# IuvenisSapiens/Qwen3-TTS-Rust

Hardware: AMD Instinct MI355X
Metric: audio-seconds generated per second (aggregate over GPUs) = concurrent real-time streams; RTF and first-chunk latency from the single-utterance leg (higher is better)
Workload: dtype i8

## Files before the change

### qwen3-tts-rust_amd/csrc/kernels.hip

```cpp
#include "kernels.h"
#include <cstdlib>
#include "q3_common.h"
#include "../../include/q3tts_spec.h"
#include "kdev.h"
#include "wslice.h"

namespace q3 {

Q3_STAMP_SETTER(set_stamp_buffer)

template <int LPR, int MT>
__global__ void __launch_bounds__(512) k_gemv_q8(Q8Mat w, int row0, int nrows, const int8_t* __restrict__ xq,
                                                 const uint16_t* __restrict__ xd, float* __restrict__ out,
                                                 int out_stride, int ntok) {
    constexpr int R = 64 / LPR, BPL = LPR / 2, NLD = 8 / BPL;
    __shared__ float red[8][R * MT];
    const int lane = threadIdx.x & 63, wave = threadIdx.x >> 6;
    const int r = lane % R, q = lane / R, half = q & 1, bil = q >> 1;
    const int nseg = w.K >> 8, nb = w.K >> 5;
    const int sseg = blockIdx.y, seg = sseg * 8 + wave;
    const int tok0 = blockIdx.z * MT;
    const bool active = seg < nseg;
    float acc[MT];
#pragma unroll
// ... 558 lines not shown
                asm volatile("" : "+v"(xl), "+v"(c) :: "memory");
                av[8 - NLATE + i] = *reinterpret_cast<const i32x4v*>(xl + (8 - NLATE + i) * 32);
            }
#pragma unroll
            for (int g4 = 0; g4 < 4; g4++) {
                const f32x2v sc_a = f32x2v{D[4 * g4], D[4 * g4 + 1]}, sc_b = f32x2v{D[4 * g4 + 2], D[4 * g4 + 3]};
                const f32x2v ca = f32x2v{(float)c[4 * g4], (float)c[4 * g4 + 1]}, cb = f32x2v{(float)c[4 * g4 + 2], (float)c[4 * g4 + 3]};
                acc2[2 * g4] = __builtin_elementwise_fma(ca, sc_a, acc2[2 * g4]);
                acc2[2 * g4 + 1] = __builtin_elementwise_fma(cb, sc_b, acc2[2 * g4 + 1]);
            }
        }
#pragma unroll
        for (int g = 0; g < 16; g++) red[wave][(g & 3) + 8 * (g >> 2) + 4 * half][r] = acc2[g >> 1][g & 1];
    };
    auto seg_sums = [&](int m, int c4) -> float4 {
        float4 v[4];
#pragma unroll
        for (int s2 = 0; s2 < 4; s2++) v[s2] = *reinterpret_cast<const float4*>(&red[s2][m][c4]);
        float4 S = v[0];
#pragma unroll
        for (int s2 = 1; s2 < 4; s2++)
            if (s2 < nsg) { S.x = S.x + v[s2].x; S.y = S.y + v[s2].y; S.z = S.z + v[s2].z; S.w = S.w + v[s2].w; }
        if (nsg > 4) {
            asm volatile("" ::: "memory");
#pragma unroll
            for (int s2 = 0; s2 < 4; s2++) v[s2] = *reinterpret_cast<const float4*>(&red[4 + s2][m][c4]);
#pragma unroll
            for (int s2 = 0; s2 < 4; s2++)
                if (4 + s2 < nsg) { S.x = S.x + v[s2].x; S.y = S.y + v[s2].y; S.z = S.z + v[s2].z; S.w = S.w + v[s2].w; }
        }
        return S;
    };
    const int nthr = 64 * (nseg < 8 ? nseg : 8);
    load_w(0, 0, 8);
    chain();
    Q3_STAMP(1);
    if (GU) { load_a(); load_w(1, 0, 8); }
    wg_barrier_lds();
    Q3_STAMP(2);
    if (!GU) {
        for (int t = threadIdx.x; t < 256; t += nthr) {
            const int m = t >> 3, c4 = (t & 7) * 4, tok = tok0 + m;
            const float4 S = seg_sums(m, c4);
            const int orow = blockIdx.x * 32 + c4;
            if (orow < nrows && tok < ntok) *reinterpret_cast<float4*>(out + ((size_t)sseg * ntok + tok) * out_stride + orow) = S;
        }
        Q3_STAMP(6);
        Q3_STAMP_FLUSH();
        return;
    }
    for (int t = threadIdx.x; t < 256; t += nthr) *reinterpret_cast<float4*>(&gate_s[4 * t]) = seg_sums(t >> 3, (t & 7) * 4);
    wg_barrier_lds();
    Q3_STAMP(3);
    chain();
    Q3_STAMP(4);
    wg_barrier_lds();
    Q3_STAMP(5);
    for (int t = threadIdx.x; t < 256; t += nthr) {
        const int m = t >> 3, c4 = (t & 7) * 4, tok = tok0 + m;
        const float4 U = seg_sums(m, c4), G = *reinterpret_cast<const float4*>(&gate_s[4 * t]);
        const float y0 = q3_swiglu(G.x, U.x), y1 = q3_swiglu(G.y, U.y), y2 = q3_swiglu(G.z, U.z), y3 = q3_swiglu(G.w, U.w);
        float amax = fmaxf(fmaxf(q3_fabsf(y0), q3_fabsf(y1)), fmaxf(q3_fabsf(y2), q3_fabsf(y3)));
        amax = fmaxf(amax, xor_lane<4>(amax)); amax = fmaxf(amax, xor_lane<2>(amax)); amax = fmaxf(amax, xor_lane<1>(amax));
        const float dd = amax / 127.0f;
        const float id = (dd != 0.0f) ? (1.0f / dd) : 0.0f;
        if (tok < ntok) {
            const uint32_t pk = ((uint32_t)(int)q3_rintf(y0 * id) & 0xFFu) | (((uint32_t)(int)q3_rintf(y1 * id) & 0xFFu) << 8) |
                                (((uint32_t)(int)q3_rintf(y2 * id) & 0xFFu) << 16) | (((uint32_t)(int)q3_rintf(y3 * id) & 0xFFu) << 24);
            *reinterpret_cast<uint32_t*>(aq + (size_t)tok * ff + blockIdx.x * 32 + c4) = pk;
            if (c4 == 0) ad[(size_t)tok * (ff >> 5) + blockIdx.x] = f2h(dd);
        }
    }
    Q3_STAMP(6);
    Q3_STAMP_FLUSH();
}

template <bool GU, int TS>
__global__ void __launch_bounds__(512) __attribute__((amdgpu_waves_per_eu(2, 2)))
k_gemm_kq_mfma(Q8Mat w, int row0, int nrows, const int8_t* __restrict__ xq, const uint16_t* __restrict__ xd, float* __restrict__ out, int out_stride,
               int ntok, int ff, int8_t* __restrict__ aq, uint16_t* __restrict__ ad) {
    __shared__ float red[8][32][33];
    __shared__ float gate_s[GU ? 4 : 1][GU ? 1024 : 1];
    const int lane = threadIdx.x & 63, wave = threadIdx.x >> 6;
    const int r = lane & 31, half = lane >> 5;
    const int nseg = w.K >> 8, nb = w.K >> 5;
    const int sseg = blockIdx.y, seg = sseg * 8 + wave;
    int nsg = nseg - sseg * 8;
    if (nsg > 8) nsg = 8;
    const bool active = seg < nseg;
    const int ntiles = (ntok + 31) >> 5;
    constexpr int NM = GU ? 2 : 1;
    const int row_first = row0 + blockIdx.x * 32;
    wslice_dispatch<TS>(w, (row_first > w.Npad - 1 ? w.Npad - 1 : row_first) >> 5, [&](auto tag) {
        constexpr int WT = decltype(tag)::value;
        constexpr bool Q5 = WT == Q3_T_Q5_K, Q6 = WT == Q3_T_Q6_K;
#pragma unroll 1
        for (int q = 0; q < NM; q++) {
            WSlice<2, WT> ws;
            ws.dwv = make_uint4(0, 0, 0, 0); ws.mv = make_uint4(0, 0, 0, 0);
            int row = row_first + r + q * ff;
            if (row > w.Npad - 1) row = w.Npad - 1;
            if (active) { ws.load(w, row >> 5, row & 31, seg, half, 0); ws.finish(half); }
            const float d0 = h2f(half_of(ws.dwv, 0)), d1 = h2f(half_of(ws.dwv, 1));
            int lt = 0;
#pragma unroll 1
            for (int tt = blockIdx.z; tt < ntiles; tt += gridDim.z, lt++) {
                const int tok0 = tt * 32;
                if (active) {
                    int atok = tok0 + r;
                    if (atok > ntok - 1) atok = ntok - 1;
                    const int8_t* xp = xq + (size_t)atok * w.K + seg * 256 + half * 16;
                    const uint4 dxa = *reinterpret_cast<const uint4*>(xd + (size_t)atok * nb + seg * 8);
                    float acc[16];
#pragma unroll
                    for (int g = 0; g < 16; g++) acc[g] = 0.0f;
                    const i32x4v ones = i32x4v{0x01010101, 0x01010101, 0x01010101, 0x01010101}, zero4 = i32x4v{0, 0, 0, 0};
#pragma unroll
                    for (int ip = 0; ip < 4; ip++) {
                        f32x32q D;
#pragma unroll
                        for (int g = 0; g < 32; g++) D[g] = 0.0f;
                        const uint32_t ex = half ? half_of(dxa, 2 * ip + 1) : half_of(dxa, 2 * ip);
                        D = __builtin_amdgcn_mfma_f32_32x32x1f32(h2f(ex), 1.0f, D, 0, 0, 0);
#pragma unroll
                        for (int i2 = 0; i2 < 2; i2++) {
                            const int i = 2 * ip + i2;
                            const i32x4v av = *reinterpret_cast<const i32x4v*>(xp + i * 32);
                            const i32x4v wv = i32x4v{(int)ws.wv[i].x, (int)ws.wv[i].y, (int)ws.wv[i].z, (int)ws.wv[i].w};
                            i32x16 z16;
#pragma unroll
                            for (int g = 0; g < 16; g++) z16[g] = 0;
                            if (Q5) {
                                const i32x16 c = __builtin_amdgcn_mfma_i32_32x32x32_i8(av, wv, z16, 0, 0, 0);
                                const i32x16 cx = __builtin_amdgcn_mfma_i32_32x32x32_i8(av, ones, z16, 0, 0, 0);
                                const int scb = ws.mbyte(i), mb = ws.mbyte(8 + i);
#pragma unroll
                                for (int g = 0; g < 16; g++) {
                                    const int i1 = __mul24(scb, c[g]), i2v = __mul24(mb, cx[g]);
                                    const float a = d0 * (float)i1;
                                    const float a2 = d1 * (float)i2v;
                                    const float diff = a - a2;
                                    acc[g] = q3_fmaf(diff, D[16 * i2 + g], acc[g]);
                                }
                            } else if (Q6) {
                                const i32x4v wlo = half ? zero4 : wv, whi = half ? wv : zero4, olo = half ? zero4 : ones, ohi = half ? ones : zero4;
                                const i32x16 clo = __builtin_amdgcn_mfma_i32_32x32x32_i8(av, wlo, z16, 0, 0, 0);
                                const i32x16 chi = __builtin_amdgcn_mfma_i32_32x32x32_i8(av, whi, z16, 0, 0, 0);
                                const i32x16 xlo = __builtin_amdgcn_mfma_i32_32x32x32_i8(av, olo, z16, 0, 0, 0);
                                const i32x16 xhi = __builtin_amdgcn_mfma_i32_32x32x32_i8(av, ohi, z16, 0, 0, 0);
                                const int s0 = (int)(int8_t)ws.mbyte(2 * i), s1 = (int)(int8_t)ws.mbyte(2 * i + 1);
#pragma unroll
                                for (int g = 0; g < 16; g++) {
                                    const int isum = __mul24(clo[g] - 32 * xlo[g], s0) + __mul24(chi[g] - 32 * xhi[g], s1);
                                    const float a = d0 * (float)isum;
                                    acc[g] = q3_fmaf(a, D[16 * i2 + g], acc[g]);
                                }
                            } else {
                                const i32x16 c = __builtin_amdgcn_mfma_i32_32x32x32_i8(av, wv, z16, 0, 0, 0);
                                const float dwf = h2f(half_of(ws.dwv, i));
#pragma unroll
                                for (int g = 0; g < 16; g++) acc[g] = q3_fmaf((float)c[g], dwf * D[16 * i2 + g], acc[g]);
                            }
                        }
                    }
#pragma unroll
                    for (int g = 0; g < 16; g++) red[wave][(g & 3) + 8 * (g >> 2) + 4 * half][r] = acc[g];
                }
                wg_barrier_lds();
                for (int t = threadIdx.x; t < 32 * 32; t += blockDim.x) {
                    const int m = t >> 5, rr = t & 31, tok = tok0 + m;
                    float v8[8];
#pragma unroll
                    for (int s2 = 0; s2 < 8; s2++) v8[s2] = red[s2][m][rr];
                    float S = v8[0];
#pragma unroll
                    for (int s2 = 1; s2 < 8; s2++) S = (s2 < nsg) ? S + v8[s2] : S;
                    if (!GU) {
                        const int orow = blockIdx.x * 32 + rr;
                        if (orow < nrows && tok < ntok) out[((size_t)sseg * ntok + tok) * out_stride + orow] = S;
                    } else if (q == 0) gate_s[lt][t] = S;
                    else {
                        const float y = q3_swiglu(gate_s[lt][t], S);
                        float amax = q3_fabsf(y);
                        amax = fmaxf(amax, xor_lane<16>(amax)); amax = fmaxf(amax, xor_lane<8>(amax)); amax = fmaxf(amax, xor_lane<4>(amax));
                        amax = fmaxf(amax, xor_lane<2>(amax)); amax = fmaxf(amax, xor_lane<1>(amax));
                        const float dd = amax / 127.0f;
                        const float id = (dd != 0.0f) ? (1.0f / dd) : 0.0f;
                        if (tok < ntok) {
                            aq[(size_t)tok * ff + blockIdx.x * 32 + rr] = (int8_t)(int)q3_rintf(y * id);
                            if (rr == 0) ad[(size_t)tok * (ff >> 5) + blockIdx.x] = f2h(dd);
                        }
                    }
                }
                wg_barrier_lds();
            }
        }
    });
}


__global__ void __launch_bounds__(64) k_rmsnorm_quant(NormArgs a) {
    const int tok = blockIdx.x, lane = threadIdx.x;
    const int nch = a.d >> 8;
    const float* hin = a.h_in;
    if (a.idx_keys) hin += (size_t)key_code(a.idx_keys[(size_t)tok * a.idx_stride]) * a.h_stride;
    else if (a.idx) hin += (size_t)a.idx[(size_t)tok * a.idx_stride] * a.h_stride;
    else hin += (size_t)tok * a.h_stride;
    float4 x[8];
    float p = 0.0f;
#pragma unroll
    for (int c = 0; c < 8; c++) {
        if (c < nch) {
            float4 v = *reinterpret_cast<const float4*>(hin + 256 * c + 4 * lane);
            if (a.nparts > 0) {
                const float* pp = a.parts + (size_t)tok * a.parts_stride + 256 * c + 4 * lane;
                float4 y = *reinterpret_cast<const float4*>(pp);
                for (int s = 1; s < a.nparts; s++) {
                    const float4 z = *reinterpret_cast<const float4*>(pp + (size_t)s * gridDim.x * a.parts_stride);
                    y.x = y.x + z.x; y.y = y.y + z.y; y.z = y.z + z.z; y.w = y.w + z.w;
                }
                v.x = v.x + y.x; v.y = v.y + y.y; v.z = v.z + y.z; v.w = v.w + y.w;
            }
            if (a.h_out) *reinterpret_cast<float4*>(a.h_out + (size_t)tok * a.d + 256 * c + 4 * lane) = v;
            x[c] = v;
            p = q3_fmaf(v.x, v.x, p); p = q3_fmaf(v.y, v.y, p); p = q3_fmaf(v.z, v.z, p); p = q3_fmaf(v.w, v.w, p);
        }
    }
    const float ss = wave_sum_bfly(p);
    const float mean = ss / (float)a.d;
    const float scale = 1.0f / q3_sqrtf(mean + a.eps);
#pragma unroll
    for (int c = 0; c < 8; c++) {
        if (c < nch) {
            const float4 g = *reinterpret_cast<const float4*>(a.g + 256 * c + 4 * lane);
            float4 y;
            y.x = (x[c].x * scale) * g.x; y.y = (x[c].y * scale) * g.y;
            y.z = (x[c].z * scale) * g.z; y.w = (x[c].w * scale) * g.w;
            if (a.xn_out) *reinterpret_cast<float4*>(a.xn_out + (size_t)tok * a.d + 256 * c + 4 * lane) = y;
            float amax = fmaxf(fmaxf(q3_fabsf(y.x), q3_fabsf(y.y)), fmaxf(q3_fabsf(y.z), q3_fabsf(y.w)));
            amax = fmaxf(amax, xor_lane<1>(amax)); amax = fmaxf(amax, xor_lane<2>(amax)); amax = fmaxf(amax, xor_lane<4>(amax));
            const float dd = amax / 127.0f;
            const float id = (dd != 0.0f) ? (1.0f / dd) : 0.0f;
            const int q0 = (int)q3_rintf(y.x * id), q1 = (int)q3_rintf(y.y * id), q2 = (int)q3_rintf(y.z * id), q3v = (int)q3_rintf(y.w * id);
            const uint32_t pk = (uint32_t)(q0 & 0xFF) | ((uint32_t)(q1 & 0xFF) << 8) | ((uint32_t)(q2 & 0xFF) << 16) | ((uint32_t)(q3v & 0xFF) << 24);
            *reinterpret_cast<uint32_t*>(a.xq + (size_t)tok * a.d + 256 * c + 4 * lane) = pk;
            if ((lane & 7) == 0) a.xd[(size_t)tok * (a.d >> 5) + 8 * c + (lane >> 3)] = f2h(dd);
        }
    }
}
void launch_rmsnorm_quant(hipStream_t st, const NormArgs& a, int ntok) {
    hipLaunchKernelGGL(k_rmsnorm_quant, dim3(ntok), dim3(64), 0, st, a);
}

__global__ void __launch_bounds__(64) k_qk_rope_append(QkvRows qkv, int n_head, int n_kv,
                                                       const float* __restrict__ q_norm_w, const float* __restrict__ k_norm_w,
                                                       float eps, const float* __restrict__ rope_cos,
                                                       const float* __restrict__ rope_sin, int n_ctx,
                                                       const int32_t* __restrict__ mrope_sec, TokMeta tm, KvCache kv,
                                                       int layer, float* __restrict__ qrot) {
    const int hv = blockIdx.x, tok = blockIdx.y, lane = threadIdx.x;
    const float* vec = qkv.row(tok) + (size_t)hv * 128;
    float x1 = vec[lane], x2 = vec[lane + 64];
    const int seq = tm.seq_of(tok), slot = tm.slot_of(tok);
    const int page = kv.page_of(seq, slot >> 6);
    const int ps = slot & 63;
    if (hv < n_head + n_kv) {
        const float* w = hv < n_head ? q_norm_w : k_norm_w;
        float p = x1 * x1;
        p = q3_fmaf(x2, x2, p);
        const float ss = wave_sum_bfly(p);
        const float mean = ss / 128.0f;
        const float scale = 1.0f / q3_sqrtf(mean + eps);
        const float y1 = (x1 * scale) * w[lane], y2 = (x2 * scale) * w[lane + 64];
        int32_t sec[4] = { mrope_sec[0], mrope_sec[1], mrope_sec[2], mrope_sec[3] };
        int pp = tm.pos_of(tok, q3_mrope_stream(lane, sec));
        if (pp < 0) pp = 0;
        if (pp > n_ctx - 1) pp = n_ctx - 1;
        float o1, o2;
        q3_rope_pair(y1, y2, rope_cos[(size_t)pp * 64 + lane], rope_sin[(size_t)pp * 64 + lane], &o1, &o2);
        if (hv < n_head) {
            float* dst = qrot + ((size_t)tok * n_head + hv) * 128;
            dst[lane] = o1; dst[lane + 64] = o2;
        } else {
            const int kh = hv - n_head;
            uint16_t* Kb = kv.k + (size_t)page * kv.page_stride() + (size_t)layer * kv.layer_stride() + (size_t)kh * 8192;
            Kb[((lane >> 3) * 64 + ps) * 8 + (lane & 7)] = f2h(o1);
            Kb[(((lane + 64) >> 3) * 64 + ps) * 8 + (lane & 7)] = f2h(o2);
        }
    } else {
        const int vh = hv - n_head - n_kv;
        uint16_t* Vb = kv.v + (size_t)page * kv.page_stride() + (size_t)layer * kv.layer_stride() + (size_t)vh * 8192;
        Vb[ps * 128 + lane] = f2h(x1);
        Vb[ps * 128 + lane + 64] = f2h(x2);
    }
}
void launch_qk_rope_append(hipStream_t st, const QkvRows& qkv, const float*, int n_head, int n_kv,
                           const float* q_norm_w, const float* k_norm_w, float eps, const float* rope_cos,
                           const float* rope_sin, int n_ctx, const int32_t* mrope_sec, const TokMeta& tm,
                           const KvCache& kv, int layer, float* qrot, int ntok) {
    hipLaunchKernelGGL(k_qk_rope_append, dim3(n_head + 2 * n_kv, ntok), dim3(64), 0, st, qkv, n_head, n_kv,
                       q_norm_w, k_norm_w, eps, rope_cos, rope_sin, n_ctx, mrope_sec, tm, kv, layer, qrot);
}

__global__ void __launch_bounds__(256) k_attention(const float* __restrict__ qrot, int n_head, int n_kv, TokMeta tm,
                                                   KvCache kv, int layer, float* __restrict__ att,
                                                   int8_t* __restrict__ aq, uint16_t* __restrict__ ad) {
    __shared__ float q_s[128];
    __shared__ float p_s[256];
    __shared__ float red_s[4][128];
    __shared__ float wmax_s[4];
    const int h = blockIdx.x, tok = blockIdx.y, tid = threadIdx.x, lane = tid & 63, wave = tid >> 6;
    const int seq = tm.seq_of(tok), n = tm.slot_of(tok) + 1;
    const int kvh = h / (n_head / n_kv);
    const size_t head_off = (size_t)layer * kv.layer_stride() + (size_t)kvh * 8192;
    if (tid < 128) q_s[tid] = qrot[((size_t)tok * n_head + h) * 128 + tid];
    __syncthreads();
    const float scale = 0.08838834764831845f;
    const int jj = lane >> 4, dc = lane & 15;
    float M = 0.0f, L = 0.0f, O[8];
#pragma unroll
    for (int i = 0; i < 8; i++) O[i] = 0.0f;
    for (int c0 = 0; c0 < n; c0 += 256) {
        const int jbase = c0 + wave * 64;
        const bool valid = (jbase + lane) < n;
        float s = -INFINITY;
        if (jbase < n) {
            const int page = kv.page_of(seq, jbase >> 6);
            const uint16_t* Kb = kv.k + (size_t)page * kv.page_stride() + head_off;
            float acc = 0.0f;
#pragma unroll
            for (int d8 = 0; d8 < 16; d8++) {
                const uint4 kk = *reinterpret_cast<const uint4*>(Kb + (d8 * 64 + lane) * 8);
                const float4 qa = *reinterpret_cast<const float4*>(&q_s[8 * d8]);
                const float4 qb = *reinterpret_cast<const float4*>(&q_s[8 * d8 + 4]);
                acc = q3_fmaf(qa.x, h2f(kk.x & 0xFFFFu), acc); acc = q3_fmaf(qa.y, h2f(kk.x >> 16), acc);
                acc = q3_fmaf(qa.z, h2f(kk.y & 0xFFFFu), acc); acc = q3_fmaf(qa.w, h2f(kk.y >> 16), acc);
                acc = q3_fmaf(qb.x, h2f(kk.z & 0xFFFFu), acc); acc = q3_fmaf(qb.y, h2f(kk.z >> 16), acc);
                acc = q3_fmaf(qb.z, h2f(kk.w & 0xFFFFu), acc); acc = q3_fmaf(qb.w, h2f(kk.w >> 16), acc);
            }
            if (valid) s = acc * scale;
        }
        const float wm = wave_max_bfly(s);
        if (lane == 0) wmax_s[wave] = wm;
        __syncthreads();
        const float mc = fmaxf(fmaxf(wmax_s[0], wmax_s[1]), fmaxf(wmax_s[2], wmax_s[3]));
        const float p = valid ? q3_expf(s - mc) : 0.0f;
        p_s[wave * 64 + lane] = p;
        __syncthreads();
        float S[8];
#pragma unroll
        for (int i = 0; i < 8; i++) S[i] = 0.0f;
        const int cn = (n - c0) < 256 ? (n - c0) : 256;
#pragma unroll 4
        for (int u = 0; u < 16; u++) {
            if (16 * u < cn) {
                const int jl = 16 * u + 4 * wave + jj;
                const int jg = c0 + jl;
                const float pj = p_s[jl];
                uint4 vv = make_uint4(0, 0, 0, 0);
                if (jg < n) {
                    const int page = kv.page_of(seq, jg >> 6);
                    vv = *reinterpret_cast<const uint4*>(kv.v + (size_t)page * kv.page_stride() + head_off + (jg & 63) * 128 + dc * 8);
                }
                S[0] = q3_fmaf(pj, h2f(vv.x & 0xFFFFu), S[0]); S[1] = q3_fmaf(pj, h2f(vv.x >> 16), S[1]);
                S[2] = q3_fmaf(pj, h2f(vv.y & 0xFFFFu), S[2]); S[3] = q3_fmaf(pj, h2f(vv.y >> 16), S[3]);
                S[4] = q3_fmaf(pj, h2f(vv.z & 0xFFFFu), S[4]); S[5] = q3_fmaf(pj, h2f(vv.z >> 16), S[5]);
                S[6] = q3_fmaf(pj, h2f(vv.w & 0xFFFFu), S[6]); S[7] = q3_fmaf(pj, h2f(vv.w >> 16), S[7]);
            }
        }
#pragma unroll
        for (int i = 0; i < 8; i++) {
            const float a = S[i] + xor_lane<16>(S[i]);
            const float T = a + xor_lane<32>(a);
            if (jj == 0) red_s[wave][dc * 8 + i] = T;
        }
        __syncthreads();
        if (wave == 0) {
            float a = p_s[lane];
            a = a + p_s[lane + 64]; a = a + p_s[lane + 128]; a = a + p_s[lane + 192];
            const float lc = wave_sum_bfly(a);
            float oc[8];
#pragma unroll
            for (int i = 0; i < 8; i++) oc[i] = (red_s[0][dc * 8 + i] + red_s[1][dc * 8 + i]) + (red_s[2][dc * 8 + i] + red_s[3][dc * 8 + i]);
            if (c0 == 0) {
                M = mc; L = lc;
#pragma unroll
                for (int i = 0; i < 8; i++) O[i] = oc[i];
            } else {
                const float mn = fmaxf(M, mc);
                const float ea = q3_expf(M - mn), eb = q3_expf(mc - mn);
                const float t = lc * eb;
                L = q3_fmaf(L, ea, t);
#pragma unroll
                for (int i = 0; i < 8; i++) { const float u2 = oc[i] * eb; O[i] = q3_fmaf(O[i], ea, u2); }
                M = mn;
            }
        }
        __syncthreads();
    }
    if (wave == 0) {
        float y[8];
        float amax = 0.0f;
#pragma unroll
        for (int i = 0; i < 8; i++) { y[i] = O[i] / L; amax = fmaxf(amax, q3_fabsf(y[i])); }
        amax = fmaxf(amax, xor_lane<1>(amax));
        amax = fmaxf(amax, xor_lane<2>(amax));
        const float dd = amax / 127.0f;
        const float id = (dd != 0.0f) ? (1.0f / dd) : 0.0f;
        if (jj == 0) {
            const size_t o = ((size_t)tok * n_head + h) * 128 + dc * 8;
            if (att) {
#pragma unroll
                for (int i = 0; i < 8; i++) att[o + i] = y[i];
            }
            uint32_t lo = 0, hi = 0;
#pragma unroll
            for (int i = 0; i < 4; i++) {
                lo |= (uint32_t)((int)q3_rintf(y[i] * id) & 0xFF) << (8 * i);
                hi |= (uint32_t)((int)q3_rintf(y[i + 4] * id) & 0xFF) << (8 * i);
            }
            *reinterpret_cast<uint2*>(aq + o) = make_uint2(lo, hi);
            if ((dc & 3) == 0) ad[o >> 5] = f2h(dd);
        }
    }
}
void launch_attention(hipStream_t st, const float* qrot, int n_head, int n_kv, const TokMeta& tm, const KvCache& kv,
                      int layer, float* att, int8_t* aq, uint16_t* ad, int ntok) {
    hipLaunchKernelGGL(k_attention, dim3(n_head, ntok), dim3(256), 0, st, qrot, n_head, n_kv, tm, kv, layer, att, aq, ad);
}

__global__ void __launch_bounds__(256) k_swiglu_quant(const float* __restrict__ gu, int ff, int8_t* __restrict__ aq,
                                                      uint16_t* __restrict__ ad) {
    const int tok = blockIdx.y;
    const int e = (blockIdx.x * 256 + threadIdx.x) * 4;
    if (e >= ff) return;
    const float4 g = *reinterpret_cast<const float4*>(gu + (size_t)tok * 2 * ff + e);
    const float4 u = *reinterpret_cast<const float4*>(gu + (size_t)tok * 2 * ff + ff + e);
    float4 y;
    y.x = q3_swiglu(g.x, u.x); y.y = q3_swiglu(g.y, u.y); y.z = q3_swiglu(g.z, u.z); y.w = q3_swiglu(g.w, u.w);
    float amax = fmaxf(fmaxf(q3_fabsf(y.x), q3_fabsf(y.y)), fmaxf(q3_fabsf(y.z), q3_fabsf(y.w)));
    amax = fmaxf(amax, xor_lane<1>(amax)); amax = fmaxf(amax, xor_lane<2>(amax)); amax = fmaxf(amax, xor_lane<4>(amax));
    const float dd = amax / 127.0f;
    const float id = (dd != 0.0f) ? (1.0f / dd) : 0.0f;
    const uint32_t pk = (uint32_t)((int)q3_rintf(y.x * id) & 0xFF) | ((uint32_t)((int)q3_rintf(y.y * id) & 0xFF) << 8) |
                        ((uint32_t)((int)q3_rintf(y.z * id) & 0xFF) << 16) | ((uint32_t)((int)q3_rintf(y.w * id) & 0xFF) << 24);
    *reinterpret_cast<uint32_t*>(aq + (size_t)tok * ff + e) = pk;
    if ((threadIdx.x & 7) == 0) ad[(size_t)tok * (ff >> 5) + (e >> 5)] = f2h(dd);
}
void launch_swiglu_quant(hipStream_t st, const float* gu, int ff, int8_t* aq, uint16_t* ad, int ntok) {
    hipLaunchKernelGGL(k_swiglu_quant, dim3((ff / 4 + 255) / 256, ntok), dim3(256), 0, st, gu, ff, aq, ad);
}

__global__ void __launch_bounds__(256) k_argmax(const float* __restrict__ logits, int stride, int start, int end,
                                                const int32_t* __restrict__ mask_per_tok, int32_t* __restrict__ out,
                                                int out_stride, int add) {
    __shared__ float bv[256];
    __shared__ int bi[256];
    const int tok = blockIdx.x, t = threadIdx.x;
    const int mask_idx = mask_per_tok ? mask_per_tok[tok] : -1;
    const float* lg = logits + (size_t)tok * stride;
    float mv = -INFINITY;
    int mi = start;
    for (int i = start + t; i < end; i += 256) {
        const float v = (i == mask_idx) ? -INFINITY : lg[i];
        if (v > mv) { mv = v; mi = i; }
    }
    bv[t] = mv; bi[t] = mi;
    __syncthreads();
    for (int s = 128; s >= 1; s >>= 1) {
        if (t < s) {
            const float v2 = bv[t + s]; const int i2 = bi[t + s];
            if (v2 > bv[t] || (v2 == bv[t] && i2 < bi[t])) { bv[t] = v2; bi[t] = i2; }
        }
        __syncthreads();
    }
    if (t == 0) out[(size_t)tok * out_stride] = bi[0] + add;
}
void launch_argmax(hipStream_t st, const float* logits, int stride, int start, int end, const int32_t* mask_per_tok,
                   int32_t* out, int out_stride, int add, int ntok) {
    hipLaunchKernelGGL(k_argmax, dim3(ntok), dim3(256), 0, st, logits, stride, start, end, mask_per_tok, out, out_stride, add);
}

__global__ void __launch_bounds__(256) k_project(const float* __restrict__ x, int x_stride, const float* __restrict__ Wt,
                                                 const float* __restrict__ b, int n_in, int n_out,
                                                 float* __restrict__ out, int out_stride) {
    extern __shared__ float xs[];
    const int tok = blockIdx.y, o = blockIdx.x * 256 + threadIdx.x;
    for (int i = threadIdx.x; i < n_in; i += 256) xs[i] = x[(size_t)tok * x_stride + i];
    __syncthreads();
    if (o >= n_out) return;
    float sum = b[o];
#pragma unroll 8
    for (int i = 0; i < n_in; i++) { const float t = xs[i] * Wt[(size_t)i * n_out + o]; sum = sum + t; }
    out[(size_t)tok * out_stride + o] = sum;
}
void launch_project(hipStream_t st, const float* x, int x_stride, const float* Wt, const float* b, int n_in, int n_out,
                    float* out, int out_stride, int ntok) {
    hipLaunchKernelGGL(k_project, dim3((n_out + 255) / 256, ntok), dim3(256), n_in * sizeof(float), st, x, x_stride, Wt, b,
                       n_in, n_out, out, out_stride);
}
template <int CT>
__global__ void __launch_bounds__(256) k_project_table(const float* __restrict__ table, int64_t rows,
                                                       const float* __restrict__ Wt, const float* __restrict__ b,
                                                       int n_in, int n_out, float* __restrict__ out) {
    extern __shared__ float xs[];
    const int64_t r0 = (int64_t)blockIdx.y * CT;
    const int o = blockIdx.x * 256 + threadIdx.x;
    for (int i = threadIdx.x; i < CT * n_in; i += 256) {
        const int64_t r = r0 + i / n_in;
        xs[i] = r < rows ? table[(size_t)r * n_in + (i % n_in)] : 0.0f;
    }
    __syncthreads();
    if (o >= n_out) return;
    float sum[CT];
#pragma unroll
    for (int c = 0; c < CT; c++) sum[c] = b[o];
    for (int i = 0; i < n_in; i++) {
        const float wv = Wt[(size_t)i * n_out + o];
#pragma unroll
        for (int c = 0; c < CT; c++) { const float t = xs[c * n_in + i] * wv; sum[c] = sum[c] + t; }
    }
#pragma unroll
    for (int c = 0; c < CT; c++) if (r0 + c < rows) out[(size_t)(r0 + c) * n_out + o] = sum[c];
}
void launch_project_table(hipStream_t st, const float* table, int64_t rows, const float* Wt, const float* b, int n_in,
                          int n_out, float* out) {
    constexpr int CT = 4;
    hipLaunchKernelGGL((k_project_table<CT>), dim3((n_out + 255) / 256, (unsigned)((rows + CT - 1) / CT)), dim3(256),
                       CT * n_in * sizeof(float), st, table, rows, Wt, b, n_in, n_out, out);
}

__global__ void __launch_bounds__(256) k_argmax_keys(const float* __restrict__ logits, int stride, int n, const int32_t* __restrict__ mask_per_tok,
                                                     unsigned long long* __restrict__ keys, int key_stride) {
    __shared__ unsigned long long best[256];
    const int tok = blockIdx.x, t = threadIdx.x;
    const int mk = mask_per_tok ? mask_per_tok[tok] : -1;
    unsigned long long k = pack_key(-INFINITY, 0);
    for (int i = t; i < n; i += 256) {
        const float v = logits[(size_t)tok * stride + i];
        if (i != mk && v > -INFINITY) { const unsigned long long c = pack_key(v, i); k = c > k ? c : k; }
    }
    best[t] = k;
    __syncthreads();
    for (int s = 128; s >= 1; s >>= 1) { if (t < s && best[t + s] > best[t]) best[t] = best[t + s]; __syncthreads(); }
    if (t == 0) keys[(size_t)tok * key_stride] = best[0];
}
void launch_argmax_keys(hipStream_t st, const float* logits, int stride, int n, const int32_t* mask_per_tok, unsigned long long* keys,
                        int key_stride, int ntok) {
    hipLaunchKernelGGL(k_argmax_keys, dim3(ntok), dim3(256), 0, st, logits, stride, n, mask_per_tok, keys, key_stride);
}


template <int TYPE>
__device__ __forceinline__ void load8(const void* row, int e, float* v) {
    if (TYPE == Q3_T_F32) {
        const float4 a = *reinterpret_cast<const float4*>((const float*)row + e), b = *reinterpret_cast<const float4*>((const float*)row + e + 4);
        v[0] = a.x; v[1] = a.y; v[2] = a.z; v[3] = a.w; v[4] = b.x; v[5] = b.y; v[6] = b.z; v[7] = b.w;
    } else {
        const uint4 u = *reinterpret_cast<const uint4*>((const uint16_t*)row + e);
        const uint32_t wds[4] = { u.x, u.y, u.z, u.w };
#pragma unroll
        for (int i = 0; i < 4; i++) {
            if (TYPE == Q3_T_BF16) { v[2 * i] = q3_bits_f32(wds[i] << 16); v[2 * i + 1] = q3_bits_f32(wds[i] & 0xFFFF0000u); }
            else { v[2 * i] = h2f(wds[i] & 0xFFFFu); v[2 * i + 1] = h2f(wds[i] >> 16); }
        }
    }
}
__device__ __forceinline__ float quad_xor1(float v) { return __int_as_float(__builtin_amdgcn_update_dpp(0, __float_as_int(v), 0xB1, 0xF, 0xF, false)); }
__device__ __forceinline__ float quad_xor2(float v) { return __int_as_float(__builtin_amdgcn_update_dpp(0, __float_as_int(v), 0x4E, 0xF, 0xF, false)); }
template <typename T> __device__ __forceinline__ float lane_bcast(float v, T lane_const) { return __int_as_float(__builtin_amdgcn_readlane(__float_as_int(v), lane_const)); }
template <int TYPE, int MT, int RW>
__global__ void __launch_bounds__(256) k_gemv_float(const void* __restrict__ w, int K, int row0, int nrows, const float* __restrict__ x,
                                                    int x_stride, float* __restrict__ out, int out_stride, int ntok) {
    const int lane = threadIdx.x & 63, wave = threadIdx.x >> 6;
    const int r0 = (blockIdx.x * 4 + wave) * RW, tok0 = blockIdx.y * MT;
    if (r0 >= nrows) return;
    const size_t esz = TYPE == Q3_T_F32 ? 4 : 2;
    const char* rows[RW];
#pragma unroll
    for (int q = 0; q < RW; q++) { const int rr = r0 + q < nrows ? r0 + q : nrows - 1; rows[q] = (const char*)w + (size_t)(row0 + rr) * K * esz; }
    const int nseg = K >> 8;
    float y[MT][RW], S[MT][RW];
#pragma unroll
    for (int m = 0; m < MT; m++)
#pragma unroll
        for (int q = 0; q < RW; q++) { y[m][q] = 0.0f; S[m][q] = 0.0f; }
    for (int e0 = 0; e0 < K; e0 += 512) {
        const int e = e0 + 8 * lane;
        float wv[RW][8];
        if (e < K) {
#pragma unroll
            for (int q = 0; q < RW; q++) load8<TYPE>(rows[q], e, wv[q]);
        }
#pragma unroll
        for (int m = 0; m < MT; m++) {
            int tok = tok0 + m;
            if (tok > ntok - 1) tok = ntok - 1;
            const float* xv = x + (size_t)tok * x_stride;
            float4 xa = make_float4(0.f, 0.f, 0.f, 0.f), xb = xa;
            if (e < K) { xa = *reinterpret_cast<const float4*>(xv + e); xb = *reinterpret_cast<const float4*>(xv + e + 4); }
#pragma unroll
            for (int q = 0; q < RW; q++) {
                float bt = 0.0f;
                if (e < K) {
                    float c = 0.0f;
                    c = q3_fmaf(wv[q][0], xa.x, c); c = q3_fmaf(wv[q][1], xa.y, c); c = q3_fmaf(wv[q][2], xa.z, c); c = q3_fmaf(wv[q][3], xa.w, c);
                    c = q3_fmaf(wv[q][4], xb.x, c); c = q3_fmaf(wv[q][5], xb.y, c); c = q3_fmaf(wv[q][6], xb.z, c); c = q3_fmaf(wv[q][7], xb.w, c);
                    const float a = c + quad_xor1(c);
                    bt = a + quad_xor2(a);
                }
#pragma unroll
                for (int sg = 0; sg < 2; sg++) {
                    const int s = (e0 >> 8) + sg;
                    if (s < nseg) {
                        float acc = 0.0f;
#pragma unroll
                        for (int j = 0; j < 8; j++) acc = acc + lane_bcast(bt, 32 * sg + 4 * j);
                        S[m][q] = (s % Q3_SSEG_SEGS == 0) ? acc : S[m][q] + acc;
                        if (s % Q3_SSEG_SEGS == Q3_SSEG_SEGS - 1 || s == nseg - 1) y[m][q] = (s < Q3_SSEG_SEGS) ? S[m][q] : y[m][q] + S[m][q];
                    }
                }
            }
        }
    }
    if (lane == 0) {
#pragma unroll
        for (int m = 0; m < MT; m++)
#pragma unroll
            for (int q = 0; q < RW; q++) if (tok0 + m < ntok && r0 + q < nrows) out[(size_t)(tok0 + m) * out_stride + r0 + q] = y[m][q];
    }
}
template <int TYPE>
static void gemv_float_mt(hipStream_t st, int mt, const FMat& w, int row0, int nrows, const float* x, int x_stride, float* out, int out_stride, int ntok) {
    dim3 grid((nrows + 3) / 4, (ntok + mt - 1) / mt);
    if (mt == 1) hipLaunchKernelGGL((k_gemv_float<TYPE, 1, 1>), grid, dim3(256), 0, st, w.w, w.K, row0, nrows, x, x_stride, out, out_stride, ntok);
    else if (mt == 2) hipLaunchKernelGGL((k_gemv_float<TYPE, 2, 1>), grid, dim3(256), 0, st, w.w, w.K, row0, nrows, x, x_stride, out, out_stride, ntok);
    else if (mt == 4) hipLaunchKernelGGL((k_gemv_float<TYPE, 4, 1>), grid, dim3(256), 0, st, w.w, w.K, row0, nrows, x, x_stride, out, out_stride, ntok);
    else hipLaunchKernelGGL((k_gemv_float<TYPE, 8, 1>), grid, dim3(256), 0, st, w.w, w.K, row0, nrows, x, x_stride, out, out_stride, ntok);
}

__device__ __forceinline__ bool xcd_tile(int n_row_tiles, int n_tok_tiles, int* row_tile, int* tok_tile) {
    const int id = blockIdx.x, xcd = id & 7, slot = id >> 3;
    *row_tile = (slot / n_tok_tiles) * 8 + xcd;
    *tok_tile = slot % n_tok_tiles;
    return *row_tile < n_row_tiles;
}
static inline unsigned xcd_grid(int n_row_tiles, int n_tok_tiles) { return (unsigned)(((n_row_tiles + 7) / 8) * 8 * n_tok_tiles); }
typedef float f32x32 __attribute__((ext_vector_type(32)));
template <int TYPE> struct RawChunk { uint4 a; };
template <> struct RawChunk<Q3_T_F32> { uint4 a, b; };
template <int TYPE>
__device__ __forceinline__ RawChunk<TYPE> load_raw(const char* p) {
    RawChunk<TYPE> r;
    r.a = *reinterpret_cast<const uint4*>(p);
    if constexpr (TYPE == Q3_T_F32) r.b = *reinterpret_cast<const uint4*>(p + 16);
    return r;
}
template <int TYPE>
__device__ __forceinline__ void unpack_raw(const RawChunk<TYPE>& r, float* v) {
    if constexpr (TYPE == Q3_T_F32) {
        v[0] = __uint_as_float(r.a.x); v[1] = __uint_as_float(r.a.y); v[2] = __uint_as_float(r.a.z); v[3] = __uint_as_float(r.a.w);
        v[4] = __uint_as_float(r.b.x); v[5] = __uint_as_float(r.b.y); v[6] = __uint_as_float(r.b.z); v[7] = __uint_as_float(r.b.w);
    } else {
        const uint32_t wds[4] = { r.a.x, r.a.y, r.a.z, r.a.w };
#pragma unroll
        for (int i = 0; i < 4; i++) {
            if constexpr (TYPE == Q3_T_BF16) { v[2 * i] = q3_bits_f32(wds[i] << 16); v[2 * i + 1] = q3_bits_f32(wds[i] & 0xFFFF0000u); }
            else { v[2 * i] = h2f(wds[i] & 0xFFFFu); v[2 * i + 1] = h2f(wds[i] >> 16); }
        }
    }
}
constexpr int FM_TOK = 32, FM_PAD = 33;
template <int TYPE>
__global__ void __launch_bounds__(512) __attribute__((amdgpu_waves_per_eu(2, 2))) k_gemm_float_mfma(const void* __restrict__ wt, int K, int tile0, int nrows, const float* __restrict__ x,
                                                         int x_stride, float* __restrict__ out, int out_stride, int ntok) {
    extern __shared__ float segsum[];
    const int lane = threadIdx.x & 63, wave = threadIdx.x >> 6;
    int tile, tt;
    if (!xcd_tile((nrows + 63) >> 6, (ntok + FM_TOK - 1) / FM_TOK, &tile, &tt)) return;
    const int tok0 = tt * FM_TOK;
    const int nseg = K >> 8;
    constexpr size_t CH = (TYPE == Q3_T_F32 ? 32 : 16) * 64;
    const char* wbase = (const char*)wt + (size_t)(tile0 + tile) * (size_t)(K >> 3) * CH + (size_t)lane * (CH / 64);
    int tok = tok0 + (lane & 31);
    if (tok > ntok - 1) tok = ntok - 1;
    const float* xrow = x + (size_t)tok * x_stride;
    const int orow = threadIdx.x & 63, otok = threadIdx.x >> 6;
    float y[4] = { 0.0f, 0.0f, 0.0f, 0.0f };
    for (int ss = 0; ss * Q3_SSEG_SEGS < nseg; ss++) {
        const int s = ss * Q3_SSEG_SEGS + wave;
        if (s < nseg) {
            f32x32 acc;
#pragma unroll
            for (int v = 0; v < 32; v++) acc[v] = 0.0f;
            const char* wp = wbase + (size_t)s * 32 * CH;
            const float* xp = xrow + (s << 8);
            RawChunk<TYPE> raw[4];
            float4 xb[8];
#pragma unroll
            for (int j = 0; j < 4; j++) raw[j] = load_raw<TYPE>(wp + (size_t)j * CH);
#pragma unroll
// ... 283 lines not shown
```

Measured before the change: 706.0.

## Prefetch K/V tiles into registers and overlap with Q handoff in decode attention

Restructures the decode attention kernel to load all K rows and the V tiles for each 256-token chunk into registers before the dot products, so global loads are in flight while Q is staged and scores are computed. It also specialises the chunk on how many 64-token pages are live, reads the page table through the constant address space, remaps heads so blocks sharing a KV head are spread out, and swaps __syncthreads for an LDS-only barrier. The aim is to hide memory latency in the latency-bound decode attention. In exchange it raises register pressure (pinned to 4 waves per EU) and grows code size through four template instantiations.

```diff
diff --git a/qwen3-tts-rust_amd/csrc/kernels.hip b/qwen3-tts-rust_amd/csrc/kernels.hip
--- a/qwen3-tts-rust_amd/csrc/kernels.hip
+++ b/qwen3-tts-rust_amd/csrc/kernels.hip
@@ -884,79 +884,126 @@
                        q_norm_w, k_norm_w, eps, rope_cos, rope_sin, n_ctx, mrope_sec, tm, kv, layer, qrot);
 }
 
-__global__ void __launch_bounds__(256) k_attention(const float* __restrict__ qrot, int n_head, int n_kv, TokMeta tm,
-                                                   KvCache kv, int layer, float* __restrict__ att,
-                                                   int8_t* __restrict__ aq, uint16_t* __restrict__ ad) {
-    __shared__ float q_s[128];
+__global__ void __launch_bounds__(256) __attribute__((amdgpu_waves_per_eu(4, 4)))
+k_attention(const float* __restrict__ qrot, int n_head, int n_kv, TokMeta tm, KvCache kv, int layer, float* __restrict__ att,
+            int8_t* __restrict__ aq, uint16_t* __restrict__ ad) {
+    __shared__ __attribute__((aligned(16))) float q_s[128];
     __shared__ float p_s[256];
     __shared__ float red_s[4][128];
     __shared__ float wmax_s[4];
-    const int h = blockIdx.x, tok = blockIdx.y, tid = threadIdx.x, lane = tid & 63, wave = tid >> 6;
+    const int tok = blockIdx.y, tid = threadIdx.x, lane = tid & 63, wave = __builtin_amdgcn_readfirstlane(tid >> 6);
+    const int grp = n_head / n_kv, bx = blockIdx.x;
+    const int h = (n_kv & 7) == 0 ? (bx % n_kv) * grp + bx / n_kv : bx;
     const int seq = tm.seq_of(tok), n = tm.slot_of(tok) + 1;
-    const int kvh = h / (n_head / n_kv);
+    const int kvh = h / grp;
     const size_t head_off = (size_t)layer * kv.layer_stride() + (size_t)kvh * 8192;
-    if (tid < 128) q_s[tid] = qrot[((size_t)tok * n_head + h) * 128 + tid];
-    __syncthreads();
+    const int jj = lane >> 4, dc = lane & 15;
+    typedef const int32_t __attribute__((address_space(4))) * const_i32_ptr;
+    const const_i32_ptr ptab = (const_i32_ptr)(uintptr_t)kv.page_table;
+    auto page_of = [&](int logical) { return kv.page_table ? ptab[(size_t)seq * kv.max_pages + logical] : seq; };
+    const float qv = qrot[((size_t)tok * n_head + h) * 128 + (tid & 127)];
     const float scale = 0.08838834764831845f;
-    const int jj = lane >> 4, dc = lane & 15;
     float M = 0.0f, L = 0.0f, O[8];
 #pragma unroll
     for (int i = 0; i < 8; i++) O[i] = 0.0f;
     for (int c0 = 0; c0 < n; c0 += 256) {
+        const int cn = (n - c0) < 256 ? (n - c0) : 256;
         const int jbase = c0 + wave * 64;
-        const bool valid = (jbase + lane) < n;
-        float s = -INFINITY;
-        if (jbase < n) {
-            const int page = kv.page_of(seq, jbase >> 6);
-            const uint16_t* Kb = kv.k + (size_t)page * kv.page_stride() + head_off;
-            float acc = 0.0f;
-#pragma unroll
-            for (int d8 = 0; d8 < 16; d8++) {
-                const uint4 kk = *reinterpret_cast<const uint4*>(Kb + (d8 * 64 + lane) * 8);
-                const float4 qa = *reinterpret_cast<const float4*>(&q_s[8 * d8]);
-                const float4 qb = *reinterpret_cast<const float4*>(&q_s[8 * d8 + 4]);
-                acc = q3_fmaf(qa.x, h2f(kk.x & 0xFFFFu), acc); acc = q3_fmaf(qa.y, h2f(kk.x >> 16), acc);
-                acc = q3_fmaf(qa.z, h2f(kk.y & 0xFFFFu), acc); acc = q3_fmaf(qa.w, h2f(kk.y >> 16), acc);
-                acc = q3_fmaf(qb.x, h2f(kk.z & 0xFFFFu), acc); acc = q3_fmaf(qb.y, h2f(kk.z >> 16), acc);
-                acc = q3_fmaf(qb.z, h2f(kk.w & 0xFFFFu), acc); acc = q3_fmaf(qb.w, h2f(kk.w >> 16), acc);
-            }
-            if (valid) s = acc * scale;
-        }
-        const float wm = wave_max_bfly(s);
-        if (lane == 0) wmax_s[wave] = wm;
-        __syncthreads();
-        const float mc = fmaxf(fmaxf(wmax_s[0], wmax_s[1]), fmaxf(wmax_s[2], wmax_s[3]));
-        const float p = valid ? q3_expf(s - mc) : 0.0f;
-        p_s[wave * 64 + lane] = p;
-        __syncthreads();
-        float S[8];
-#pragma unroll
-        for (int i = 0; i < 8; i++) S[i] = 0.0f;
-        const int cn = (n - c0) < 256 ? (n - c0) : 256;
-#pragma unroll 4
-        for (int u = 0; u < 16; u++) {
-            if (16 * u < cn) {
-                const int jl = 16 * u + 4 * wave + jj;
-                const int jg = c0 + jl;
-                const float pj = p_s[jl];
-                uint4 vv = make_uint4(0, 0, 0, 0);
-                if (jg < n) {
-                    const int page = kv.page_of(seq, jg >> 6);
-                    vv = *reinterpret_cast<const uint4*>(kv.v + (size_t)page * kv.page_stride() + head_off + (jg & 63) * 128 + dc * 8);
+        float S[8], mc;
+        auto chunk = [&](auto nb_const) {
+            constexpr int NB = decltype(nb_const)::value;
+            uint4 vreg[4 * NB];
+            int pg[NB];
+#pragma unroll
+            for (int b = 0; b < NB; b++) pg[b] = page_of((c0 >> 6) + b);
+            auto load_v = [&](int b, const float* after) {
+                const uint16_t* Vb = kv.v + (size_t)pg[b] * kv.page_stride() + head_off;
+#pragma unroll
+                for (int g = 0; g < 4; g++) {
+                    const int jg = c0 + 64 * b + 16 * g + 4 * wave + jj;
+                    uint32_t off = (uint32_t)(((jg < n ? jg : n - 1) & 63) * 128 + dc * 8);
+                    if (after) asm volatile("" : "+v"(off) : "v"(*after));
+                    vreg[4 * b + g] = *reinterpret_cast<const uint4*>(Vb + off);
                 }
-                S[0] = q3_fmaf(pj, h2f(vv.x & 0xFFFFu), S[0]); S[1] = q3_fmaf(pj, h2f(vv.x >> 16), S[1]);
-                S[2] = q3_fmaf(pj, h2f(vv.y & 0xFFFFu), S[2]); S[3] = q3_fmaf(pj, h2f(vv.y >> 16), S[3]);
-                S[4] = q3_fmaf(pj, h2f(vv.z & 0xFFFFu), S[4]); S[5] = q3_fmaf(pj, h2f(vv.z >> 16), S[5]);
-                S[6] = q3_fmaf(pj, h2f(vv.w & 0xFFFFu), S[6]); S[7] = q3_fmaf(pj, h2f(vv.w >> 16), S[7]);
-            }
-        }
+            };
+            auto q_handoff = [&]() {
+                if (c0 == 0) {
+                    q_s[tid & 127] = qv;
+                    wg_barrier_lds();
+                }
+            };
+            const bool valid = (jbase + lane) < n;
+            float s = -INFINITY;
+            if (jbase < n) {
+                int pgk = pg[0];
+#pragma unroll
+                for (int b = 1; b < NB; b++) pgk = wave == b ? pg[b] : pgk;
+                const uint16_t* Kb = kv.k + (size_t)pgk * kv.page_stride() + head_off;
+                uint4 kreg[16];
+#pragma unroll
+                for (int d8 = 0; d8 < 16; d8++) kreg[d8] = *reinterpret_cast<const uint4*>(Kb + (d8 * 64 + lane) * 8);
+                load_v(0, nullptr);
+                q_handoff();
+                float acc = 0.0f;
+                float4 qa = *reinterpret_cast<const float4*>(&q_s[0]), qb = *reinterpret_cast<const float4*>(&q_s[4]);
+#pragma unroll
+                for (int d8 = 0; d8 < 16; d8++) {
+                    const uint4 kk = kreg[d8];
+                    float4 na = qa, nb = qb;
+                    if (d8 < 15) {
+                        int qi = 8 * (d8 + 1);
+                        asm volatile("" : "+v"(qi) : "v"(acc));
+                        na = *reinterpret_cast<const float4*>(&q_s[qi]);
+                        nb = *reinterpret_cast<const float4*>(&q_s[qi + 4]);
+                    }
+                    acc = q3_fmaf(qa.x, h2f(kk.x & 0xFFFFu), acc); acc = q3_fmaf(qa.y, h2f(kk.x >> 16), acc);
+                    acc = q3_fmaf(qa.z, h2f(kk.y & 0xFFFFu), acc); acc = q3_fmaf(qa.w, h2f(kk.y >> 16), acc);
+                    acc = q3_fmaf(qb.x, h2f(kk.z & 0xFFFFu), acc); acc = q3_fmaf(qb.y, h2f(kk.z >> 16), acc);
+                    acc = q3_fmaf(qb.z, h2f(kk.w & 0xFFFFu), acc); acc = q3_fmaf(qb.w, h2f(kk.w >> 16), acc);
+                    qa = na; qb = nb;
+                }
+                if (valid) s = acc * scale;
+            } else {
+                load_v(0, nullptr);
+                q_handoff();
+            }
+#pragma unroll
+            for (int b = 1; b < NB; b++) load_v(b, &s);
+            const float wm = wave_max_bfly(s);
+            if (lane == 0) wmax_s[wave] = wm;
+            wg_barrier_lds();
+            mc = fmaxf(fmaxf(wmax_s[0], wmax_s[1]), fmaxf(wmax_s[2], wmax_s[3]));
+            const float p = valid ? q3_expf(s - mc) : 0.0f;
+            p_s[wave * 64 + lane] = p;
+            wg_barrier_lds();
+#pragma unroll
+            for (int i = 0; i < 8; i++) S[i] = 0.0f;
+#pragma unroll
+            for (int u = 0; u < 4 * NB; u++) {
+                if (16 * u < cn) {
+                    const int jl = 16 * u + 4 * wave + jj;
+                    const int jg = c0 + jl;
+                    const float pj = p_s[jl];
+                    uint4 vv = vreg[u];
+                    if (!(jg < n)) vv = make_uint4(0, 0, 0, 0);
+                    S[0] = q3_fmaf(pj, h2f(vv.x & 0xFFFFu), S[0]); S[1] = q3_fmaf(pj, h2f(vv.x >> 16), S[1]);
+                    S[2] = q3_fmaf(pj, h2f(vv.y & 0xFFFFu), S[2]); S[3] = q3_fmaf(pj, h2f(vv.y >> 16), S[3]);
+                    S[4] = q3_fmaf(pj, h2f(vv.z & 0xFFFFu), S[4]); S[5] = q3_fmaf(pj, h2f(vv.z >> 16), S[5]);
+                    S[6] = q3_fmaf(pj, h2f(vv.w & 0xFFFFu), S[6]); S[7] = q3_fmaf(pj, h2f(vv.w >> 16), S[7]);
+                }
+            }
+        };
+        if (cn <= 64) chunk(std::integral_constant<int, 1>());
+        else if (cn <= 128) chunk(std::integral_constant<int, 2>());
+        else if (cn <= 192) chunk(std::integral_constant<int, 3>());
+        else chunk(std::integral_constant<int, 4>());
 #pragma unroll
         for (int i = 0; i < 8; i++) {
             const float a = S[i] + xor_lane<16>(S[i]);
             const float T = a + xor_lane<32>(a);
             if (jj == 0) red_s[wave][dc * 8 + i] = T;
         }
-        __syncthreads();
+        wg_barrier_lds();
         if (wave == 0) {
             float a = p_s[lane];
             a = a + p_s[lane + 64]; a = a + p_s[lane + 128]; a = a + p_s[lane + 192];
@@ -978,7 +1025,7 @@
                 M = mn;
             }
         }
-        __syncthreads();
+        wg_barrier_lds();
     }
     if (wave == 0) {
         float y[8];
```

After: 721.0, median of 6. +2.1%, better.
